# steineggerlab/folddisco

Measured on AMD Instinct MI355X. Metric: structures/sec indexed, higher is better.
Workload: dtype f32+u32; 1 GPU; Swiss-Prot scale: 542000 synthetic AFDB-shaped structures (175035960 residues, 17705019118 postings, 26085150307 value bytes) index build, PDBTrRosetta default; 1 rank(s), contiguous id ranges, per rank 1 build call(s) of <= 542000 structures: one resident index, no merge; structures=542000, structures_per_gpu=542000, residues=175035960, postings=17705019118, parallelism=shard-by-structure x1, build_calls_per_rank=1

## Files before the change

folddisco_amd/csrc/k_hash.hip:

```cpp
#include "fd_device.h"
#include "fd_geom_other.h"
#ifndef FD_EMIT_WAVES
#define FD_EMIT_WAVES 5
#endif
#define FD_MSD_BUCKETS 40u

__global__ __launch_bounds__(FD_WAVE) void k_pair_count(fd_batch_view B, fd_hash_consts C, uint32_t *__restrict__ counts) {
    uint32_t w = fd_xcd_remap(blockIdx.x, B.n_work);
    if (w >= B.n_work) return;
    const uint32_t s = B.wi_struct[w];
    const uint32_t r0 = B.res_off[s], r1 = B.res_off[s + 1];
    const uint32_t i = B.wi_i0[w] + threadIdx.x;
    const bool vi = i < r1 && B.hash_ok[i];
    fd_v3 cai = {0.f, 0.f, 0.f};
    if (vi) cai = fd_load3(B.ca_xyz, i);
    uint32_t cnt = 0;
    for (uint32_t j = r0; j < r1; ++j) {
        if (!B.hash_ok[j]) continue;
        fd_v3 caj = fd_load3(B.ca_xyz, j);
        float d2 = fd_dist2(cai, caj);
        cnt += (vi && i != j && !(d2 > C.d2_max)) ? 1u : 0u;
    }
    for (int off = 32; off > 0; off >>= 1) cnt += __shfl_down(cnt, off, FD_WAVE);
    if (threadIdx.x == 0 && cnt) atomicAdd(&counts[s], cnt);
}

template <bool WRITE_IDS>
__device__ __forceinline__ void drain(const fd_batch_view &B, const fd_hash_consts &C, const uint32_t *q, uint32_t n,
                                      uint32_t i0, uint32_t r0, uint32_t s, uint32_t id, const uint64_t *seg_off,
                                      uint32_t *cursor, uint32_t *keys, uint32_t *ids) {
    const uint32_t lane = threadIdx.x;
    uint32_t base = 0;
    if (lane == 0) base = atomicAdd(&cursor[s], n);
    base = __shfl(base, 0, FD_WAVE);
    if (lane < n) {
        uint32_t e = q[lane];
        uint32_t i = i0 + (e >> 16), j = r0 + (e & 0xffffu);
        fd_v3 n1 = fd_load3(B.n_xyz, i), ca1 = fd_load3(B.ca_xyz, i), cb1 = fd_load3(B.cb_xyz, i);
        fd_v3 n2 = fd_load3(B.n_xyz, j), ca2 = fd_load3(B.ca_xyz, j), cb2 = fd_load3(B.cb_xyz, j);
        fd_feature f = fd_pair_feature(n1, ca1, cb1, n2, ca2, cb2);
        uint32_t h = fd_hash_enc(B.aa[i], B.aa[j], f, C.q);
        uint64_t pos = seg_off[s] + base + lane;
        keys[pos] = h;
        if (WRITE_IDS) ids[pos] = id;
    }
}

template <bool WRITE_IDS>
__global__ __launch_bounds__(FD_WAVE) void k_pair_emit(fd_batch_view B, fd_hash_consts C, const uint64_t *__restrict__ seg_off,
                                                       uint32_t *__restrict__ cursor, uint32_t *__restrict__ keys,
                                                       uint32_t *__restrict__ ids, uint32_t first_id) {
    __shared__ uint32_t q[2 * FD_WAVE];
    uint32_t w = fd_xcd_remap(blockIdx.x, B.n_work);
    if (w >= B.n_work) return;
    const uint32_t s = B.wi_struct[w];
    const uint32_t r0 = B.res_off[s], r1 = B.res_off[s + 1];
    const uint32_t i0 = B.wi_i0[w];
    const uint32_t lane = threadIdx.x;
    const uint32_t i = i0 + lane;
    const bool vi = i < r1 && B.hash_ok[i];
    fd_v3 cai = {0.f, 0.f, 0.f};
    if (vi) cai = fd_load3(B.ca_xyz, i);
    uint32_t qn = 0;
    for (uint32_t j = r0; j < r1; ++j) {
        if (!B.hash_ok[j]) continue;
        fd_v3 caj = fd_load3(B.ca_xyz, j);
        float d2 = fd_dist2(cai, caj);
        bool pass = vi && i != j && !(d2 > C.d2_max);
        uint64_t m = __ballot(pass);
        if (m == 0) continue;
        if (pass) q[qn + fd_mbcnt(m)] = (lane << 16) | (j - r0);
        qn += (uint32_t)__popcll(m);
        if (qn >= FD_WAVE) {
            __syncthreads();
            qn -= FD_WAVE;
            drain<WRITE_IDS>(B, C, q + qn, FD_WAVE, i0, r0, s, first_id + s, seg_off, cursor, keys, ids);
            __syncthreads();
        }
    }
    if (qn) {
        __syncthreads();
        drain<WRITE_IDS>(B, C, q, qn, i0, r0, s, first_id + s, seg_off, cursor, keys, ids);
    }
}

__global__ __launch_bounds__(256) void k_frames(fd_batch_view B, uint32_t n_res, fd_frame *__restrict__ frames) {
    uint32_t r = blockIdx.x * blockDim.x + threadIdx.x;
    if (r >= n_res) return;
    fd_frame F;
    if (B.hash_ok[r]) F = fd_make_frame(fd_load3(B.n_xyz, r), fd_load3(B.ca_xyz, r), fd_load3(B.cb_xyz, r));
    else { F = fd_frame{}; F.ca = fd_load3(B.ca_xyz, r); }
    F.pad = __uint_as_float((uint32_t)B.aa[r]);
    frames[r] = F;
}

typedef float fd_f2 __attribute__((ext_vector_type(2)));
#define FD_NOT_HASHABLE 0x100u

__device__ __forceinline__ bool fd_lane_of(uint64_t m) { return __builtin_amdgcn_inverse_ballot_w64(m); }

template <bool TYPES, class Step, class RunEnd>
__device__ __forceinline__ void fd_filter_block(const fd_batch_view &B, float d2_max, const fd_v3 &cai, uint64_t vim, uint32_t i0, uint32_t jb, uint32_t r1,
                                                float *s_cj, Step &&step, RunEnd &&run_end) {
    const uint32_t lane = threadIdx.x;
    const uint32_t jl = jb + lane;
    fd_v3 cj = {0.f, 0.f, 0.f};
    uint32_t kind = FD_NOT_HASHABLE;
    if (jl < r1) {
        cj = fd_load3(B.ca_xyz, jl);
        if (B.hash_ok[jl]) kind = TYPES ? (uint32_t)B.aa[jl] : 0u;
    }
    fd_wave_lds_fence();
    s_cj[lane] = cj.x; s_cj[FD_WAVE + lane] = cj.y; s_cj[2 * FD_WAVE + lane] = cj.z;
    fd_wave_lds_fence();
    const uint64_t okm = __ballot(kind != FD_NOT_HASHABLE);
    const uint64_t starts = __ballot(kind != (uint32_t)__shfl_up((int)kind, 1, FD_WAVE)) | 1ull;
    const bool last_block = jb + FD_WAVE >= r1;
    const uint32_t nk = okm ? 64u - (uint32_t)__builtin_clzll(okm) : 0u;
    const uint32_t nkf = (last_block && nk == 0) ? 1u : nk;
    const bool first = jb == i0;
    const fd_f2 ax = {cai.x, cai.x}, ay = {cai.y, cai.y}, az = {cai.z, cai.z};
    uint32_t k = 0;
    while (k < nkf) {
        const uint32_t t = (uint32_t)__builtin_amdgcn_readlane((int)kind, (int)k);
        const uint64_t rest = (starts >> k) >> 1;
        uint32_t ke = rest ? k + 1u + (uint32_t)__builtin_ctzll(rest) : (uint32_t)FD_WAVE;
        ke = ke < nkf ? ke : nkf;
        const bool run_last = last_block && ke >= nkf;
        const bool dead = t == FD_NOT_HASHABLE;
        if (dead && !run_last) { k = ke; continue; }
        const uint64_t vr = dead ? 0ull : vim;
        uint64_t gt = first ? (1ull << k) - 1ull : ~0ull;
        do {
            const fd_f2 xj = {s_cj[k], s_cj[k + 1]}, yj = {s_cj[FD_WAVE + k], s_cj[FD_WAVE + k + 1]}, zj = {s_cj[2 * FD_WAVE + k], s_cj[2 * FD_WAVE + k + 1]};
            const fd_f2 dx = ax - xj, dy = ay - yj, dz = az - zj;
            const fd_f2 d2 = (dx * dx + dy * dy) + dz * dz;
            const uint64_t gt1 = gt << 1 | 1ull;
            const uint64_t m0 = __ballot(!(d2.x > d2_max)) & vr & gt;
            const uint64_t m1 = (k + 1u < ke) ? (__ballot(!(d2.y > d2_max)) & vr & gt1) : 0ull;
            gt = gt1 << 1 | 1ull;
            const uint32_t k0 = k;
            k += 2;
            step(k0, t, m0, m1, run_last && k >= ke);
        } while (k < ke);
        k = ke;
        run_end(t);
    }
}

__global__ __launch_bounds__(FD_WAVE) void k_pair_count2(fd_batch_view B, fd_hash_consts C, uint32_t *__restrict__ counts) {
    __shared__ float s_cj[3 * FD_WAVE + 1];
    uint32_t w = fd_xcd_remap(blockIdx.x, B.n_work);
    if (w >= B.n_work) return;
    const uint32_t s = B.wi_struct[w];
    const uint32_t r1 = B.res_off[s + 1];
    const uint32_t i0 = B.wi_i0[w];
    const uint32_t i = i0 + threadIdx.x;
    const bool vi = i < r1 && B.hash_ok[i];
    fd_v3 cai = {0.f, 0.f, 0.f};
    if (vi) cai = fd_load3(B.ca_xyz, i);
    const uint64_t vim = __ballot(vi);
    uint32_t cnt = 0;
    for (uint32_t jb = i0; jb < r1; jb += FD_WAVE)
        fd_filter_block<false>(B, C.d2_max, cai, vim, i0, jb, r1, s_cj,
                               [&](uint32_t, uint32_t, uint64_t m0, uint64_t m1, bool) { cnt += (fd_lane_of(m0) ? 1u : 0u) + (fd_lane_of(m1) ? 1u : 0u); },
                               [](uint32_t) {});
    cnt *= 2u;
    for (int off = 32; off > 0; off >>= 1) cnt += __shfl_down(cnt, off, FD_WAVE);
    if (threadIdx.x == 0 && cnt) atomicAdd(&counts[s], cnt);
}

__global__ __launch_bounds__(256) void k_frames_perm(fd_batch_view B, fd_frame *__restrict__ frames, float *__restrict__ ca_perm, uint8_t *__restrict__ ok_perm,
                                                     uint8_t *__restrict__ aa_perm, unsigned long long *__restrict__ wide_flag) {
    __shared__ uint32_t cnt[32], cur[32];
    const uint32_t s = blockIdx.x;
    const uint32_t r0 = B.res_off[s], r1 = B.res_off[s + 1];
    if (threadIdx.x < 32) cnt[threadIdx.x] = 0;
    __syncthreads();
    for (uint32_t r = r0 + threadIdx.x; r < r1; r += 256) {
        const uint32_t a = B.aa[r];
        atomicAdd(&cnt[(B.hash_ok[r] && a < 20u) ? a : 20u], 1u);
    }
    __syncthreads();
    if (threadIdx.x == 0) { uint32_t run = 0; for (int k = 0; k < 21; ++k) { cur[k] = run; run += cnt[k]; } }
    __syncthreads();
    for (uint32_t r = r0 + threadIdx.x; r < r1; r += 256) {
        const uint32_t a = B.aa[r];
        bool ok = B.hash_ok[r] != 0;
        if (ok && a >= 20u) {
            ok = false;
            if (wide_flag) atomicOr(wide_flag, 1ull);
        }
        const uint32_t p = r0 + atomicAdd(&cur[(ok && a < 20u) ? a : 20u], 1u);
        fd_frame F;
        const fd_v3 ca = fd_load3(B.ca_xyz, r);
        if (ok) F = fd_make_frame(fd_load3(B.n_xyz, r), ca, fd_load3(B.cb_xyz, r));
        else { F = fd_frame{}; F.ca = ca; }
        F.pad = __uint_as_float(a);
        frames[p] = F;
        ca_perm[3ull * p] = ca.x; ca_perm[3ull * p + 1] = ca.y; ca_perm[3ull * p + 2] = ca.z;
        ok_perm[p] = ok ? 1 : 0;
        aa_perm[p] = (uint8_t)a;
    }
}

__global__ __launch_bounds__(FD_WAVE) void k_pair_count_msd(fd_batch_view B, fd_hash_consts C, uint32_t *__restrict__ counts) {
    __shared__ uint32_t s_cnt[FD_WAVE];
    __shared__ float s_cj[3 * FD_WAVE + 1];
    uint32_t w = fd_xcd_remap(blockIdx.x, B.n_work);
    if (w >= B.n_work) return;
    const uint32_t s = B.wi_struct[w];
    const uint32_t r1 = B.res_off[s + 1];
    const uint32_t i0 = B.wi_i0[w];
    const uint32_t lane = threadIdx.x;
    const uint32_t i = i0 + lane;
    const bool vi = i < r1 && B.hash_ok[i];
    fd_v3 cai = {0.f, 0.f, 0.f};
    uint32_t aai = 0;
    if (vi) { cai = fd_load3(B.ca_xyz, i); aai = B.aa[i]; }
    s_cnt[lane] = 0;
    __syncthreads();
    const uint64_t vim = __ballot(vi);
    uint32_t c_lo = 0, c_hi = 0, run = 0;
    const uint32_t hi_i = aai >> 4;
    for (uint32_t jb = i0; jb < r1; jb += FD_WAVE)
        fd_filter_block<true>(B, C.d2_max, cai, vim, i0, jb, r1, s_cj,
                              [&](uint32_t, uint32_t, uint64_t m0, uint64_t m1, bool) { run += (fd_lane_of(m0) ? 1u : 0u) + (fd_lane_of(m1) ? 1u : 0u); },
                              [&](uint32_t t) {
                                  if (t >= 16u) c_hi += run; else c_lo += run;
                                  if (run) atomicAdd(&s_cnt[(t * 2u + hi_i) & (FD_WAVE - 1u)], run);
                                  run = 0;
                              });
    if (c_lo) atomicAdd(&s_cnt[aai * 2u], c_lo);
    if (c_hi) atomicAdd(&s_cnt[aai * 2u + 1u], c_hi);
    __syncthreads();
    if (lane < FD_MSD_BUCKETS && s_cnt[lane]) atomicAdd(&counts[(uint64_t)lane * B.n_struct + s], s_cnt[lane]);
}

__device__ __forceinline__ fd_frame load_frame(const fd_frame *__restrict__ frames, uint32_t r) {
    const float4 *p = reinterpret_cast<const float4 *>(frames + r);
    float4 a = p[0], b = p[1], c = p[2], d = p[3], e = p[4];
    fd_frame F;
    F.ca = {a.x, a.y, a.z}; F.cb = {a.w, b.x, b.y}; F.r1 = {b.z, b.w, c.x}; F.t1 = {c.y, c.z, c.w};
    F.s2 = {d.x, d.y, d.z}; F.nv2 = {d.w, e.x, e.y}; F.len = e.z; F.pad = e.w;
    return F;
}

__device__ __attribute__((noinline)) uint2 pair_both_tab_exact(const fd_frame *__restrict__ frames, uint32_t i, uint32_t j, uint32_t aai,
                                                               uint32_t aaj, float dist_disc, float ang_disc, const uint32_t *tab) {
    fd_frame Fi = load_frame(frames, i), Fj = load_frame(frames, j);
    fd_quant q;
    q.dist_disc = dist_disc; q.ang_disc = ang_disc; q.ang2_disc = 0.0f; q.type = FD_HASH_PDBTR;
    uint32_t a, b;
    fd_pair_both_tab(Fi, Fj, aai, aaj, q, tab, &a, &b);
    return make_uint2(a, b);
}

template <int TAB, bool IDS16, bool MSD, bool DT = false>
__device__ __forceinline__ void drain2(const fd_batch_view &B, const fd_frame *__restrict__ frames, const fd_hash_consts &C,
                                       const uint32_t *tab, const uint32_t *q, uint32_t n, uint32_t i0, uint32_t r0, uint32_t s, uint32_t id,
                                       const uint64_t *seg_off, uint32_t *cursor, uint32_t *keys, void *ids, const float4 *s_fi,
                                       uint32_t *s_bc, uint64_t *s_bb, const uint64_t *s_boff) {
    const uint32_t lane = threadIdx.x;
    uint32_t base = 0, gb = 0, slots = 0;
    if (!MSD) {
        if (lane == 0) base = atomicAdd(&cursor[s], 2u * n);
        base = __shfl(base, 0, FD_WAVE);
    } else {
        s_bc[lane] = 0;
        fd_wave_lds_fence();
        if (lane < n) {
            const uint32_t e = q[lane], il = (e >> 16) & 63u, aj = e >> 22;
            const uint32_t ai = TAB == 2 ? __float_as_uint(s_fi[256 + il].w) : (uint32_t)B.aa[i0 + il];
            const uint32_t bf = ai * 2u + (aj >> 4), br = aj * 2u + (ai >> 4);
            slots = atomicAdd(&s_bc[bf], 1u) | atomicAdd(&s_bc[br], 1u) << 8 | bf << 16 | br << 24;
        }
        fd_wave_lds_fence();
        if (lane < FD_MSD_BUCKETS) { const uint32_t c = s_bc[lane]; if (c) gb = atomicAdd(&cursor[(uint64_t)lane * B.n_struct + s], c); }
    }
    uint32_t h_ij = 0, h_ji = 0, aai = 0, aaj = 0;
    if (lane < n) {
        uint32_t e = q[lane];
        uint32_t i = i0 + ((e >> 16) & 63u), j = r0 + (e & 0xffffu);
        if (TAB == 2) {
            const uint32_t il = (e >> 16) & 63u;
            const float4 a4 = s_fi[il], b4 = s_fi[64 + il], c4 = s_fi[128 + il], d4 = s_fi[192 + il], e4 = s_fi[256 + il];
            fd_frame Fi;
            Fi.ca = {a4.x, a4.y, a4.z}; Fi.cb = {a4.w, b4.x, b4.y}; Fi.r1 = {b4.z, b4.w, c4.x}; Fi.t1 = {c4.y, c4.z, c4.w};
            Fi.s2 = {d4.x, d4.y, d4.z}; Fi.nv2 = {d4.w, e4.x, e4.y}; Fi.len = e4.z; Fi.pad = e4.w;
            fd_frame Fj = load_frame(frames, j);
            aai = __float_as_uint(Fi.pad); aaj = __float_as_uint(Fj.pad);
#if defined(FD_EMIT_STUB) && FD_EMIT_STUB == 1
            h_ij = aai << 25 | aaj << 20 | (__float_as_uint(Fj.ca.x) & 0xfffffu); h_ji = aaj << 25 | aai << 20 | (__float_as_uint(Fi.ca.x) & 0xfffffu);
            if (false)
#endif
            if (!fd_pair_both_spec<DT>(Fi, Fj, aai, aaj, C.q, tab, tab + 32, &h_ij, &h_ji, tab + 64)) {
                uint2 h = pair_both_tab_exact(frames, i, j, B.aa[i], B.aa[j], C.q.dist_disc, C.q.ang_disc, tab);
                h_ij = h.x; h_ji = h.y;
                if (C.spec_miss) atomicAdd(C.spec_miss, 1ull);
            }
        } else if (TAB == 1) {
            uint2 h = pair_both_tab_exact(frames, i, j, B.aa[i], B.aa[j], C.q.dist_disc, C.q.ang_disc, tab);
            h_ij = h.x; h_ji = h.y;
        } else {
            fd_frame Fi = load_frame(frames, i), Fj = load_frame(frames, j);
            fd_pair_both(Fi, Fj, B.aa[i], B.aa[j], C.q, &h_ij, &h_ji);
        }
    }
    if (MSD) {
        if (lane < FD_MSD_BUCKETS) s_bb[lane] = s_boff[lane] + gb;
        fd_wave_lds_fence();
        if (lane < n) {
            const uint32_t sf = slots & 255u, sr = (slots >> 8) & 255u, bf = (slots >> 16) & 255u, br = slots >> 24;
            if ((((h_ij | h_ji) >> 30) || (h_ij >> 24) != bf || (h_ji >> 24) != br) && C.wide_flag) atomicOr(C.wide_flag, 1ull);
            const uint64_t pf = s_bb[bf] + sf, pr = s_bb[br] + sr;
            keys[pf] = (h_ij << 24) | s;
            keys[pr] = (h_ji << 24) | s;
            ((uint16_t *)ids)[pf] = (uint16_t)(h_ij >> 8);
            ((uint16_t *)ids)[pr] = (uint16_t)(h_ji >> 8);
        }
        return;
    }
    if (lane < n) {
        const uint64_t so = seg_off[s];
        uint64_t pos = so * C.seg_mul + (uint64_t)C.seg_cfg * (seg_off[s + 1] - so) + base + lane;
        if (IDS16) {
            if (((h_ij | h_ji) >> 30) && C.wide_flag) atomicOr(C.wide_flag, 1ull);
            uint32_t hi = s >> 16;
            uint16_t lo = (uint16_t)(s & 0xffffu);
            keys[pos] = (h_ij << 2) | hi;
            keys[pos + n] = (h_ji << 2) | hi;
            ((uint16_t *)ids)[pos] = lo;
            ((uint16_t *)ids)[pos + n] = lo;
        } else {
            keys[pos] = h_ij;
            keys[pos + n] = h_ji;
            ((uint32_t *)ids)[pos] = id;
            ((uint32_t *)ids)[pos + n] = id;
        }
    }
}

template <int TAB, bool IDS16, bool MSD, bool DT = false>
__global__ __launch_bounds__(FD_WAVE, FD_EMIT_WAVES) void k_pair_emit2(fd_batch_view B, const fd_frame *__restrict__ frames, fd_hash_consts C,
                                                        const uint64_t *__restrict__ seg_off, uint32_t *__restrict__ cursor,
                                                        uint32_t *__restrict__ keys, void *__restrict__ ids, uint32_t first_id) {
    __shared__ uint32_t q[3 * FD_WAVE];
    __shared__ float s_cj[3 * FD_WAVE + 1];
    __shared__ uint32_t tab[DT ? 64 + FD_DIST_NTHR + 1 : 64];
    uint32_t w = fd_xcd_remap(blockIdx.x, B.n_work);
    if (w >= B.n_work) return;
    if (TAB) {
        if (DT && threadIdx.x < FD_DIST_NTHR) tab[64 + threadIdx.x] = fd_dist_thr_bits[threadIdx.x];
        if (threadIdx.x == 0) {
            fd_fill_bintab(tab);
            for (int k = 0; k < FD_BINTAB_WORDS; ++k) tab[32 + k] = tab[k];
            for (int m = 0; m < 4; ++m)
                for (int k = 0; k < 4; ++k) { uint32_t v = tab[32 + 7 + 5 * m + k]; tab[32 + 7 + 5 * m + k] = v > 0x7f7fffffu ? 0x7f7fffffu : v; }
        }
        __syncthreads();
    }
    const uint32_t s = B.wi_struct[w];
    const uint32_t r0 = B.res_off[s], r1 = B.res_off[s + 1];
    const uint32_t i0 = B.wi_i0[w];
    const uint32_t lane = threadIdx.x;
    const uint32_t i = i0 + lane;
    const bool vi = i < r1 && B.hash_ok[i];
    fd_v3 cai = {0.f, 0.f, 0.f};
    if (vi) cai = fd_load3(B.ca_xyz, i);
    __shared__ float4 s_fi[5 * FD_WAVE];
    if (TAB == 2 && i < r1) {
        const float4 *fp = reinterpret_cast<const float4 *>(frames + i);
#pragma unroll
        for (int k = 0; k < 5; ++k) s_fi[k * FD_WAVE + lane] = fp[k];
    }
    __shared__ uint32_t s_bc[MSD ? FD_WAVE : 1];
    __shared__ uint64_t s_bb[MSD ? FD_MSD_BUCKETS : 1], s_boff[MSD ? FD_MSD_BUCKETS : 1];
    if (MSD && lane < FD_MSD_BUCKETS) s_boff[lane] = seg_off[(uint64_t)lane * B.n_struct + s];
    __syncthreads();
    const uint64_t vim = __ballot(vi);
    const uint32_t lane16 = lane << 16;
    uint32_t qn = 0;
    for (uint32_t jb = i0; jb < r1; jb += FD_WAVE) {
        const uint32_t jrel = jb - r0;
        fd_filter_block<MSD>(B, C.d2_max, cai, vim, i0, jb, r1, s_cj,
            [&](uint32_t k, uint32_t t, uint64_t m0, uint64_t m1, bool last) {
                const uint32_t tag = (MSD ? t << 22 : 0u) | (jrel + k);
                if (m0) {
                    if (fd_lane_of(m0)) q[__builtin_amdgcn_mbcnt_hi((uint32_t)(m0 >> 32), __builtin_amdgcn_mbcnt_lo((uint32_t)m0, qn))] = lane16 | tag;
                    qn += (uint32_t)__popcll(m0);
                }
                if (m1) {
                    if (fd_lane_of(m1)) q[__builtin_amdgcn_mbcnt_hi((uint32_t)(m1 >> 32), __builtin_amdgcn_mbcnt_lo((uint32_t)m1, qn))] = lane16 | (tag + 1u);
                    qn += (uint32_t)__popcll(m1);
                }
                while (qn >= FD_WAVE || (last && qn)) {
                    fd_wave_lds_fence();
                    uint32_t n = qn < FD_WAVE ? qn : FD_WAVE;
                    qn -= n;
                    drain2<TAB, IDS16, MSD, DT>(B, frames, C, tab, q + qn, n, i0, r0, s, first_id + s, seg_off, cursor, keys, ids, s_fi, s_bc, s_bb, s_boff);
                    fd_wave_lds_fence();
                }
            },
            [](uint32_t) {});
    }
}

__global__ __launch_bounds__(FD_WAVE) void k_row_count(fd_batch_view B, fd_hash_consts C, uint32_t *__restrict__ row_cnt, float cutoff) {
    uint32_t w = fd_xcd_remap(blockIdx.x, B.n_work);
    if (w >= B.n_work) return;
    const uint32_t s = B.wi_struct[w];
    const uint32_t r0 = B.res_off[s], r1 = B.res_off[s + 1];
    const uint32_t i = B.wi_i0[w] + threadIdx.x;
    if (i >= r1) return;
    if (fd_own_descriptor(C.q.type)) {
        uint32_t cnt = 0;
        if (B.aa[i] != 255)
            for (uint32_t j = r0; j < r1; ++j)
                cnt += (j != i && B.aa[j] != 255 && fd_accept_other(C.q.type, B, r0, r1, i, j, cutoff)) ? 1u : 0u;
        row_cnt[i] = cnt;
        return;
    }
    const bool vi = B.hash_ok[i];
    fd_v3 cai = fd_load3(B.ca_xyz, i);
    uint32_t cnt = 0;
    for (uint32_t j = r0; j < r1; ++j) {
        if (!B.hash_ok[j]) continue;
        float d2 = fd_dist2(cai, fd_load3(B.ca_xyz, j));
        cnt += (vi && i != j && !(d2 > C.d2_max)) ? 1u : 0u;
    }
    row_cnt[i] = cnt;
}

__global__ __launch_bounds__(FD_WAVE) void k_row_emit(fd_batch_view B, fd_hash_consts C, const uint64_t *__restrict__ row_off,
                                                      uint32_t *__restrict__ keys, float cutoff, uint32_t *__restrict__ ids, uint32_t first_id, int ids_partner) {
    uint32_t w = fd_xcd_remap(blockIdx.x, B.n_work);
    if (w >= B.n_work) return;
    const uint32_t s = B.wi_struct[w];
    const uint32_t r0 = B.res_off[s], r1 = B.res_off[s + 1];
    const uint32_t i = B.wi_i0[w] + threadIdx.x;
    if (i >= r1) return;
    if (fd_own_descriptor(C.q.type)) {
        if (B.aa[i] == 255) return;
        uint64_t pos = row_off[i];
        float f[FD_NFEAT];
        for (uint32_t j = r0; j < r1; ++j) {
            if (j == i || B.aa[j] == 255 || !fd_feature_other(C.q.type, B, r0, r1, i, j, cutoff, f)) continue;
            if (ids) ids[pos] = ids_partner ? j : first_id + s;
            keys[pos++] = fd_hash_other(C.q.type, f, C.q);
        }
        return;
    }
    if (!B.hash_ok[i]) return;
    fd_v3 n1 = fd_load3(B.n_xyz, i), ca1 = fd_load3(B.ca_xyz, i), cb1 = fd_load3(B.cb_xyz, i);
    uint32_t aa1 = B.aa[i];
    uint64_t pos = row_off[i];
    for (uint32_t j = r0; j < r1; ++j) {
        if (!B.hash_ok[j] || i == j) continue;
        fd_v3 ca2 = fd_load3(B.ca_xyz, j);
        if (fd_dist2(ca1, ca2) > C.d2_max) continue;
        fd_v3 n2 = fd_load3(B.n_xyz, j), cb2 = fd_load3(B.cb_xyz, j);
        fd_feature f = fd_pair_feature(n1, ca1, cb1, n2, ca2, cb2);
        if (ids) ids[pos] = ids_partner ? j : first_id + s;
        keys[pos++] = fd_hash_enc(aa1, B.aa[j], f, C.q);
    }
}

__global__ void k_hash_ok(const uint8_t *__restrict__ aa, const uint8_t *__restrict__ cb_valid, uint8_t *__restrict__ ok, uint64_t n) {
    uint64_t k = (uint64_t)blockIdx.x * blockDim.x + threadIdx.x;
    if (k < n) ok[k] = (aa[k] != 255 && (cb_valid == nullptr || cb_valid[k])) ? 1 : 0;
}

__global__ void k_selfcheck(fd_quant q, uint32_t *__restrict__ out ) {
    if (threadIdx.x != 0 || blockIdx.x != 0) return;
    const fd_v3 N[3] = {{6.661f, 8.291f, 43.860f}, {10.483f, 7.756f, 49.260f}, {5.260f, -1.068f, 41.296f}};
    const fd_v3 CA[3] = {{6.994f, 8.354f, 42.405f}, {9.429f, 7.479f, 48.266f}, {5.547f, 0.158f, 42.050f}};
    const fd_v3 CB[3] = {{8.251f, 7.488f, 42.026f}, {10.033f, 6.489f, 47.255f}, {5.773f, 1.360f, 41.130f}};
    const uint32_t AA[3] = {8u, 3u, 15u};
    const int PI[6] = {1, 1, 0, 0, 2, 2}, PJ[6] = {0, 2, 1, 2, 1, 0};
    uint32_t tab[64 + FD_DIST_NTHR + 1];
    fd_fill_bintab(tab);
    for (int k = 0; k < FD_BINTAB_WORDS; ++k) tab[32 + k] = tab[k];
    for (int m = 0; m < 4; ++m)
        for (int k = 0; k < 4; ++k) { uint32_t v = tab[32 + 7 + 5 * m + k]; tab[32 + 7 + 5 * m + k] = v > 0x7f7fffffu ? 0x7f7fffffu : v; }
    for (int k = 0; k < FD_DIST_NTHR; ++k) tab[64 + k] = fd_dist_thr_bits[k];
    fd_frame F[3];
    for (int r = 0; r < 3; ++r) F[r] = fd_make_frame(N[r], CA[r], CB[r]);
    for (int k = 0; k < 6; ++k) {
        const int i = PI[k], j = PJ[k];
        out[k] = fd_hash_pdbtr(AA[i], AA[j], fd_pair_feature(N[i], CA[i], CB[i], N[j], CA[j], CB[j]), q);
        uint32_t a, b;
        fd_pair_both_tab(F[i], F[j], AA[i], AA[j], q, tab, &a, &b);
        out[6 + k] = a;
        if (!fd_pair_both_spec(F[i], F[j], AA[i], AA[j], q, tab, tab + 32, &a, &b)) fd_pair_both_tab(F[i], F[j], AA[i], AA[j], q, tab, &a, &b);
        out[12 + k] = a;
        if (!fd_pair_both_spec<true>(F[i], F[j], AA[i], AA[j], q, tab, tab + 32, &a, &b, tab + 64)) fd_pair_both_tab(F[i], F[j], AA[i], AA[j], q, tab, &a, &b);
        out[18 + k] = a;
    }
}

extern "C++" {
void fd_launch_selfcheck(const fd_quant &q, uint32_t *out, hipStream_t st) { hipLaunchKernelGGL(k_selfcheck, dim3(1), dim3(64), 0, st, q, out); }
void fd_launch_hash_ok(const uint8_t *aa, const uint8_t *cb_valid, uint8_t *ok, uint64_t n, hipStream_t st) {
    if (!n) return;
    hipLaunchKernelGGL(k_hash_ok, dim3((unsigned)((n + 255) / 256)), dim3(256), 0, st, aa, cb_valid, ok, n);
}
static inline unsigned grid_for(uint32_t n_work) { return ((n_work + 7u) / 8u) * 8u; }
void fd_launch_pair_count(const fd_batch_view &B, const fd_hash_consts &C, uint32_t *counts, hipStream_t st) {
    if (!B.n_work) return;
    hipLaunchKernelGGL(k_pair_count, dim3(grid_for(B.n_work)), dim3(FD_WAVE), 0, st, B, C, counts);
}
void fd_launch_pair_emit(const fd_batch_view &B, const fd_hash_consts &C, const uint64_t *seg_off, uint32_t *cursor,
                         uint32_t *keys, uint32_t *ids, uint32_t first_id, hipStream_t st) {
    if (!B.n_work) return;
    if (ids)
        hipLaunchKernelGGL(k_pair_emit<true>, dim3(grid_for(B.n_work)), dim3(FD_WAVE), 0, st, B, C, seg_off, cursor, keys, ids, first_id);
    else
        hipLaunchKernelGGL(k_pair_emit<false>, dim3(grid_for(B.n_work)), dim3(FD_WAVE), 0, st, B, C, seg_off, cursor, keys, ids, first_id);
}
void fd_launch_frames(const fd_batch_view &B, uint64_t n_res, void *frames, hipStream_t st) {
    if (!n_res) return;
    hipLaunchKernelGGL(k_frames, dim3((unsigned)((n_res + 255) / 256)), dim3(256), 0, st, B, (uint32_t)n_res, (fd_frame *)frames);
}
void fd_launch_pair_count2(const fd_batch_view &B, const fd_hash_consts &C, uint32_t *counts, hipStream_t st) {
    if (!B.n_work) return;
    hipLaunchKernelGGL(k_pair_count2, dim3(grid_for(B.n_work)), dim3(FD_WAVE), 0, st, B, C, counts);
}
void fd_launch_pair_emit2(const fd_batch_view &B, const void *frames, const fd_hash_consts &C, const uint64_t *seg_off, uint32_t *cursor,
                          uint32_t *keys, void *ids, bool ids16, uint32_t first_id, hipStream_t st) {
    if (!B.n_work) return;
    dim3 g(grid_for(B.n_work)), b(FD_WAVE);
    const fd_frame *F = (const fd_frame *)frames;
    if (C.use_tab >= 2 && ids16) hipLaunchKernelGGL((k_pair_emit2<2, true, false>), g, b, 0, st, B, F, C, seg_off, cursor, keys, ids, first_id);
    else if (C.use_tab >= 2) hipLaunchKernelGGL((k_pair_emit2<2, false, false>), g, b, 0, st, B, F, C, seg_off, cursor, keys, ids, first_id);
    else if (C.use_tab && ids16) hipLaunchKernelGGL((k_pair_emit2<1, true, false>), g, b, 0, st, B, F, C, seg_off, cursor, keys, ids, first_id);
    else if (C.use_tab) hipLaunchKernelGGL((k_pair_emit2<1, false, false>), g, b, 0, st, B, F, C, seg_off, cursor, keys, ids, first_id);
    else if (ids16) hipLaunchKernelGGL((k_pair_emit2<0, true, false>), g, b, 0, st, B, F, C, seg_off, cursor, keys, ids, first_id);
    else hipLaunchKernelGGL((k_pair_emit2<0, false, false>), g, b, 0, st, B, F, C, seg_off, cursor, keys, ids, first_id);
}
void fd_launch_frames_perm(const fd_batch_view &B, void *frames, float *ca_perm, uint8_t *ok_perm, uint8_t *aa_perm, unsigned long long *wide_flag, hipStream_t st) {
    if (!B.n_struct) return;
    hipLaunchKernelGGL(k_frames_perm, dim3(B.n_struct), dim3(256), 0, st, B, (fd_frame *)frames, ca_perm, ok_perm, aa_perm, wide_flag);
}
void fd_launch_pair_count_msd(const fd_batch_view &B, const fd_hash_consts &C, uint32_t *counts, hipStream_t st) {
    if (!B.n_work) return;
    hipLaunchKernelGGL(k_pair_count_msd, dim3(grid_for(B.n_work)), dim3(FD_WAVE), 0, st, B, C, counts);
}
void fd_launch_pair_emit_msd(const fd_batch_view &B, const void *frames, const fd_hash_consts &C, const uint64_t *seg_off, uint32_t *cursor, uint32_t *keys,
                             uint16_t *ids, hipStream_t st) {
    if (!B.n_work) return;
    dim3 g(grid_for(B.n_work)), b(FD_WAVE);
    const fd_frame *F = (const fd_frame *)frames;
    if (C.use_tab == 3) hipLaunchKernelGGL((k_pair_emit2<2, true, true, true>), g, b, 0, st, B, F, C, seg_off, cursor, keys, (void *)ids, 0u);
    else if (C.use_tab == 2) hipLaunchKernelGGL((k_pair_emit2<2, true, true>), g, b, 0, st, B, F, C, seg_off, cursor, keys, (void *)ids, 0u);
    else if (C.use_tab) hipLaunchKernelGGL((k_pair_emit2<1, true, true>), g, b, 0, st, B, F, C, seg_off, cursor, keys, (void *)ids, 0u);
    else hipLaunchKernelGGL((k_pair_emit2<0, true, true>), g, b, 0, st, B, F, C, seg_off, cursor, keys, (void *)ids, 0u);
}
void fd_launch_row_count(const fd_batch_view &B, const fd_hash_consts &C, uint32_t *row_cnt, float cutoff, hipStream_t st) {
    if (!B.n_work) return;
    hipLaunchKernelGGL(k_row_count, dim3(grid_for(B.n_work)), dim3(FD_WAVE), 0, st, B, C, row_cnt, cutoff);
}
void fd_launch_row_emit(const fd_batch_view &B, const fd_hash_consts &C, const uint64_t *row_off, uint32_t *keys, float cutoff, uint32_t *ids,
                        uint32_t first_id, hipStream_t st, int ids_partner) {
    if (!B.n_work) return;
    hipLaunchKernelGGL(k_row_emit, dim3(grid_for(B.n_work)), dim3(FD_WAVE), 0, st, B, C, row_off, keys, cutoff, ids, first_id, ids_partner);
}
}
```

Before: 1.482 million structures/s.

## Count pair neighbors from global CA loads instead of LDS staging with ballots

```diff
diff --git a/folddisco_amd/csrc/fd_pair_filter.h b/folddisco_amd/csrc/fd_pair_filter.h
--- /dev/null
+++ b/folddisco_amd/csrc/fd_pair_filter.h
@@ -0,0 +1,13 @@
+#pragma once
+#include "fd_geom.h"
+
+typedef float fd_f2 __attribute__((vector_size(8)));
+
+#define FD_COUNT_UNROLL 4
+
+template <class T> FD_HD T fd_filter_d2(T ax, T ay, T az, T xj, T yj, T zj) {
+    const T dx = ax - xj, dy = ay - yj, dz = az - zj;
+    return (dx * dx + dy * dy) + dz * dz;
+}
+
+FD_HD bool fd_filter_pass(float d2, float d2_max) { return !(d2 > d2_max); }
diff --git a/folddisco_amd/csrc/k_hash.hip b/folddisco_amd/csrc/k_hash.hip
--- a/folddisco_amd/csrc/k_hash.hip
+++ b/folddisco_amd/csrc/k_hash.hip
@@ -1,5 +1,6 @@
 #include "fd_device.h"
 #include "fd_geom_other.h"
+#include "fd_pair_filter.h"
 #ifndef FD_EMIT_WAVES
 #define FD_EMIT_WAVES 5
 #endif
@@ -94,50 +95,70 @@
     frames[r] = F;
 }
 
-typedef float fd_f2 __attribute__((ext_vector_type(2)));
 #define FD_NOT_HASHABLE 0x100u
 
 __device__ __forceinline__ bool fd_lane_of(uint64_t m) { return __builtin_amdgcn_inverse_ballot_w64(m); }
+
+template <bool TYPES>
+__device__ __forceinline__ uint32_t fd_load_kind(const fd_batch_view &B, uint32_t jl, uint32_t r1) {
+    uint32_t kind = FD_NOT_HASHABLE;
+    if (jl < r1) {
+        const uint32_t a = TYPES ? (uint32_t)B.aa[jl] : 0u;
+        kind = B.hash_ok[jl] ? a : FD_NOT_HASHABLE;
+    }
+    return kind;
+}
+
+struct fd_block_runs { uint64_t starts; uint32_t nk; };
+
+__device__ __forceinline__ fd_block_runs fd_block_runs_of(uint32_t kind) {
+    const uint64_t okm = __ballot(kind != FD_NOT_HASHABLE);
+    fd_block_runs r;
+    r.starts = __ballot(kind != (uint32_t)__shfl_up((int)kind, 1, FD_WAVE)) | 1ull;
+    r.nk = okm ? 64u - (uint32_t)__builtin_clzll(okm) : 0u;
+    return r;
+}
+
+__device__ __forceinline__ uint32_t fd_run_end(const fd_block_runs &r, uint32_t k, uint32_t nk) {
+    const uint64_t rest = (r.starts >> k) >> 1;
+    const uint32_t ke = rest ? k + 1u + (uint32_t)__builtin_ctzll(rest) : (uint32_t)FD_WAVE;
+    return ke < nk ? ke : nk;
+}
+
+__device__ __forceinline__ fd_f2 fd_lds_d2x2(const float *s_cj, uint32_t k, fd_f2 ax, fd_f2 ay, fd_f2 az) {
+    const fd_f2 xj = {s_cj[k], s_cj[k + 1]}, yj = {s_cj[FD_WAVE + k], s_cj[FD_WAVE + k + 1]}, zj = {s_cj[2 * FD_WAVE + k], s_cj[2 * FD_WAVE + k + 1]};
+    return fd_filter_d2<fd_f2>(ax, ay, az, xj, yj, zj);
+}
 
 template <bool TYPES, class Step, class RunEnd>
 __device__ __forceinline__ void fd_filter_block(const fd_batch_view &B, float d2_max, const fd_v3 &cai, uint64_t vim, uint32_t i0, uint32_t jb, uint32_t r1,
                                                 float *s_cj, Step &&step, RunEnd &&run_end) {
-    const uint32_t lane = threadIdx.x;
-    const uint32_t jl = jb + lane;
+    const uint32_t lane = threadIdx.x, jl = jb + lane;
+    const uint32_t kind = fd_load_kind<TYPES>(B, jl, r1);
     fd_v3 cj = {0.f, 0.f, 0.f};
-    uint32_t kind = FD_NOT_HASHABLE;
-    if (jl < r1) {
-        cj = fd_load3(B.ca_xyz, jl);
-        if (B.hash_ok[jl]) kind = TYPES ? (uint32_t)B.aa[jl] : 0u;
-    }
+    if (jl < r1) cj = fd_load3(B.ca_xyz, jl);
     fd_wave_lds_fence();
     s_cj[lane] = cj.x; s_cj[FD_WAVE + lane] = cj.y; s_cj[2 * FD_WAVE + lane] = cj.z;
     fd_wave_lds_fence();
-    const uint64_t okm = __ballot(kind != FD_NOT_HASHABLE);
-    const uint64_t starts = __ballot(kind != (uint32_t)__shfl_up((int)kind, 1, FD_WAVE)) | 1ull;
+    const fd_block_runs R = fd_block_runs_of(kind);
     const bool last_block = jb + FD_WAVE >= r1;
-    const uint32_t nk = okm ? 64u - (uint32_t)__builtin_clzll(okm) : 0u;
-    const uint32_t nkf = (last_block && nk == 0) ? 1u : nk;
+    const uint32_t nkf = (last_block && R.nk == 0) ? 1u : R.nk;
     const bool first = jb == i0;
     const fd_f2 ax = {cai.x, cai.x}, ay = {cai.y, cai.y}, az = {cai.z, cai.z};
     uint32_t k = 0;
     while (k < nkf) {
         const uint32_t t = (uint32_t)__builtin_amdgcn_readlane((int)kind, (int)k);
-        const uint64_t rest = (starts >> k) >> 1;
-        uint32_t ke = rest ? k + 1u + (uint32_t)__builtin_ctzll(rest) : (uint32_t)FD_WAVE;
-        ke = ke < nkf ? ke : nkf;
+        const uint32_t ke = fd_run_end(R, k, nkf);
         const bool run_last = last_block && ke >= nkf;
         const bool dead = t == FD_NOT_HASHABLE;
         if (dead && !run_last) { k = ke; continue; }
         const uint64_t vr = dead ? 0ull : vim;
         uint64_t gt = first ? (1ull << k) - 1ull : ~0ull;
         do {
-            const fd_f2 xj = {s_cj[k], s_cj[k + 1]}, yj = {s_cj[FD_WAVE + k], s_cj[FD_WAVE + k + 1]}, zj = {s_cj[2 * FD_WAVE + k], s_cj[2 * FD_WAVE + k + 1]};
-            const fd_f2 dx = ax - xj, dy = ay - yj, dz = az - zj;
-            const fd_f2 d2 = (dx * dx + dy * dy) + dz * dz;
+            const fd_f2 d2 = fd_lds_d2x2(s_cj, k, ax, ay, az);
             const uint64_t gt1 = gt << 1 | 1ull;
-            const uint64_t m0 = __ballot(!(d2.x > d2_max)) & vr & gt;
-            const uint64_t m1 = (k + 1u < ke) ? (__ballot(!(d2.y > d2_max)) & vr & gt1) : 0ull;
+            const uint64_t m0 = __ballot(fd_filter_pass(d2[0], d2_max)) & vr & gt;
+            const uint64_t m1 = (k + 1u < ke) ? (__ballot(fd_filter_pass(d2[1], d2_max)) & vr & gt1) : 0ull;
             gt = gt1 << 1 | 1ull;
             const uint32_t k0 = k;
             k += 2;
@@ -148,23 +169,75 @@
     }
 }
 
+__device__ __forceinline__ bool fd_ca_pass(const float *c, const fd_v3 &a, float d2_max) {
+    return fd_filter_pass(fd_filter_d2<float>(a.x, a.y, a.z, c[0], c[1], c[2]), d2_max);
+}
+
+struct fd_ca_trip { float v[3 * FD_COUNT_UNROLL]; };
+__device__ __forceinline__ fd_ca_trip fd_load_ca_trip(const float *ca) {
+    fd_ca_trip r;
+#pragma unroll
+    for (int c = 0; c < 3 * FD_COUNT_UNROLL; ++c) r.v[c] = ca[c];
+    return r;
+}
+
+template <bool FIRST>
+__device__ __forceinline__ uint32_t fd_count_run(const float *ca, float d2_max, const fd_v3 &cai, uint32_t k, uint32_t ke) {
+    const int lane = (int)threadIdx.x;
+    uint32_t n = 0;
+    if (k + FD_COUNT_UNROLL <= ke) {
+        fd_ca_trip cur = fd_load_ca_trip(ca + 3u * k);
+        for (;;) {
+            const bool more = k + 2 * FD_COUNT_UNROLL <= ke;
+            fd_ca_trip nxt = cur;
+            if (more) nxt = fd_load_ca_trip(ca + 3u * (k + FD_COUNT_UNROLL));
+            const int rel = lane - (int)k;
+#pragma unroll
+            for (int c = 0; c < FD_COUNT_UNROLL; ++c) n += (fd_ca_pass(cur.v + 3 * c, cai, d2_max) && (!FIRST || rel < c)) ? 1u : 0u;
+            k += FD_COUNT_UNROLL;
+            if (!more) break;
+            cur = nxt;
+        }
+    }
+#pragma clang loop vectorize(disable) unroll(disable)
+    for (; k < ke; ++k)
+        n += (fd_ca_pass(ca + 3u * k, cai, d2_max) && (!FIRST || lane < (int)k)) ? 1u : 0u;
+    return n;
+}
+
+template <class RunEnd>
+__device__ __forceinline__ void fd_count_block(uint32_t kind, const float *ca, float d2_max, const fd_v3 &cai, bool vi, bool first, RunEnd &&run_end) {
+    const fd_block_runs R = fd_block_runs_of(kind);
+    uint32_t k = 0;
+    while (k < R.nk) {
+        const uint32_t t = (uint32_t)__builtin_amdgcn_readlane((int)kind, (int)k);
+        const uint32_t ke = fd_run_end(R, k, R.nk);
+        if (t != FD_NOT_HASHABLE) {
+            const uint32_t n = first ? fd_count_run<true>(ca, d2_max, cai, k, ke) : fd_count_run<false>(ca, d2_max, cai, k, ke);
+            run_end(t, vi ? n : 0u);
+        }
+        k = ke;
+    }
+}
+
 __global__ __launch_bounds__(FD_WAVE) void k_pair_count2(fd_batch_view B, fd_hash_consts C, uint32_t *__restrict__ counts) {
-    __shared__ float s_cj[3 * FD_WAVE + 1];
     uint32_t w = fd_xcd_remap(blockIdx.x, B.n_work);
     if (w >= B.n_work) return;
     const uint32_t s = B.wi_struct[w];
     const uint32_t r1 = B.res_off[s + 1];
     const uint32_t i0 = B.wi_i0[w];
-    const uint32_t i = i0 + threadIdx.x;
-    const bool vi = i < r1 && B.hash_ok[i];
+    const uint32_t lane = threadIdx.x;
+    const uint32_t i = i0 + lane;
+    uint32_t nx = fd_load_kind<false>(B, i, r1);
+    const bool vi = nx != FD_NOT_HASHABLE;
     fd_v3 cai = {0.f, 0.f, 0.f};
-    if (vi) cai = fd_load3(B.ca_xyz, i);
-    const uint64_t vim = __ballot(vi);
+    if (i < r1) cai = fd_load3(B.ca_xyz, i);
     uint32_t cnt = 0;
-    for (uint32_t jb = i0; jb < r1; jb += FD_WAVE)
-        fd_filter_block<false>(B, C.d2_max, cai, vim, i0, jb, r1, s_cj,
-                               [&](uint32_t, uint32_t, uint64_t m0, uint64_t m1, bool) { cnt += (fd_lane_of(m0) ? 1u : 0u) + (fd_lane_of(m1) ? 1u : 0u); },
-                               [](uint32_t) {});
+    for (uint32_t jb = i0; jb < r1; jb += FD_WAVE) {
+        const uint32_t kind = nx;
+        if (jb + FD_WAVE < r1) nx = fd_load_kind<false>(B, jb + FD_WAVE + lane, r1);
+        fd_count_block(kind, B.ca_xyz + 3ull * jb, C.d2_max, cai, vi, jb == i0, [&](uint32_t, uint32_t n) { cnt += n; });
+    }
     cnt *= 2u;
     for (int off = 32; off > 0; off >>= 1) cnt += __shfl_down(cnt, off, FD_WAVE);
     if (threadIdx.x == 0 && cnt) atomicAdd(&counts[s], cnt);
@@ -206,7 +279,6 @@
 
 __global__ __launch_bounds__(FD_WAVE) void k_pair_count_msd(fd_batch_view B, fd_hash_consts C, uint32_t *__restrict__ counts) {
     __shared__ uint32_t s_cnt[FD_WAVE];
-    __shared__ float s_cj[3 * FD_WAVE + 1];
     uint32_t w = fd_xcd_remap(blockIdx.x, B.n_work);
     if (w >= B.n_work) return;
     const uint32_t s = B.wi_struct[w];
@@ -214,25 +286,26 @@
     const uint32_t i0 = B.wi_i0[w];
     const uint32_t lane = threadIdx.x;
     const uint32_t i = i0 + lane;
-    const bool vi = i < r1 && B.hash_ok[i];
+    uint32_t nx = fd_load_kind<true>(B, i, r1);
+    const bool vi = nx != FD_NOT_HASHABLE;
+    const uint32_t aai = vi ? nx : 0u;
     fd_v3 cai = {0.f, 0.f, 0.f};
-    uint32_t aai = 0;
-    if (vi) { cai = fd_load3(B.ca_xyz, i); aai = B.aa[i]; }
+    if (i < r1) cai = fd_load3(B.ca_xyz, i);
     s_cnt[lane] = 0;
     __syncthreads();
-    const uint64_t vim = __ballot(vi);
-    uint32_t c_lo = 0, c_hi = 0, run = 0;
+    uint32_t c_lo = 0, c_hi = 0;
     const uint32_t hi_i = aai >> 4;
-    for (uint32_t jb = i0; jb < r1; jb += FD_WAVE)
-        fd_filter_block<true>(B, C.d2_max, cai, vim, i0, jb, r1, s_cj,
-                              [&](uint32_t, uint32_t, uint64_t m0, uint64_t m1, bool) { run += (fd_lane_of(m0) ? 1u : 0u) + (fd_lane_of(m1) ? 1u : 0u); },
-                              [&](uint32_t t) {
-                                  if (t >= 16u) c_hi += run; else c_lo += run;
-                                  if (run) atomicAdd(&s_cnt[(t * 2u + hi_i) & (FD_WAVE - 1u)], run);
-                                  run = 0;
-                              });
-    if (c_lo) atomicAdd(&s_cnt[aai * 2u], c_lo);
-    if (c_hi) atomicAdd(&s_cnt[aai * 2u + 1u], c_hi);
+    for (uint32_t jb = i0; jb < r1; jb += FD_WAVE) {
+        const uint32_t kind = nx;
+        if (jb + FD_WAVE < r1) nx = fd_load_kind<true>(B, jb + FD_WAVE + lane, r1);
+        fd_count_block(kind, B.ca_xyz + 3ull * jb, C.d2_max, cai, vi, jb == i0,
+                       [&](uint32_t t, uint32_t n) {
+                           if (t >= 16u) c_hi += n; else c_lo += n;
+                           if (n) atomicAdd(&s_cnt[(t * 2u + hi_i) & (FD_WAVE - 1u)], n);
+                       });
+    }
+    if (c_lo) atomicAdd(&s_cnt[(aai * 2u) & (FD_WAVE - 1u)], c_lo);
+    if (c_hi) atomicAdd(&s_cnt[(aai * 2u + 1u) & (FD_WAVE - 1u)], c_hi);
     __syncthreads();
     if (lane < FD_MSD_BUCKETS && s_cnt[lane]) atomicAdd(&counts[(uint64_t)lane * B.n_struct + s], s_cnt[lane]);
 }
```

Result: no change. 1.492 million structures/s (median of 6 runs) (+0.7%).
